# ZJU-FAST-Lab/Dftpav

Hardware: AMD Instinct MI355X
Metric: trajectory solves/sec (batched), 16-piece MINCO (higher is better)
Workload: dtype f64

## Files before the change

### dftpav_amd/csrc/quad_common.h

```cpp
#pragma once
#include "ref_order_common.h"

namespace dftpav {
namespace reford {

__device__ __forceinline__ double row_chain16(double acc, double v) {
  const double one = 1.0;
  asm volatile("s_nop 1\n\t" DFTPAV_FMAC_BCAST16 : "+v"(acc) : "v"(v), "v"(one));
  return acc;
}
__device__ __forceinline__ double row_add_lane0(double acc, double v) {
  const double one = 1.0;
  asm volatile("s_nop 1\n\t" DFTPAV_FMAC_BCAST(0) : "+v"(acc) : "v"(v), "v"(one));
  return acc;
}
__device__ __forceinline__ double row_max16(double v) {
  v = fmax(v, mov_dpp<0xB1>(v));
  v = fmax(v, mov_dpp<0x4E>(v));
  v = fmax(v, mov_dpp<0x141>(v));
  v = fmax(v, mov_dpp<0x140>(v));
  return v;
}
template <int CTRL> __device__ __forceinline__ double nb_dpp(double v) {
  int lo = __double2loint(v), hi = __double2hiint(v);
  lo = __builtin_amdgcn_update_dpp(0, lo, CTRL, 0xf, 0xf, true);
  hi = __builtin_amdgcn_update_dpp(0, hi, CTRL, 0xf, 0xf, true);
  return __hiloint2double(hi, lo);
}


constexpr int kDense = 24;
static_assert(kDense <= 32, "a lane's slots of the list are the bits of a 32-bit mask (solver_ref4.hip: mine |= 1u << e)");
struct DenseLds {
  ldsi_t id;
  ldsd_t s1;
  ldsd_t pl;
  ldsd_t out;
};
__host__ __device__ inline size_t q4_dense_bytes() { return ((size_t)kDense * (4 + 8 + 32 + 120) + 15) & ~(size_t)15; }
__device__ inline void q4_carve_dense(DenseLds &d, char *base) {
  ldsd_t p = (ldsd_t)reinterpret_cast<double *>(base);
  d.s1 = p; p += kDense;
  d.pl = p; p += 4 * kDense;
  d.out = p; p += 15 * kDense;
  d.id = (ldsi_t)p;
}

}
}
```

### dftpav_amd/csrc/solver_ref4.hip

```cpp
#include <hip/hip_runtime.h>
#include <cstdio>
#include <cstdlib>
#include <algorithm>

#include "ref_order_common.h"
#include "quad_common.h"

namespace dftpav {
namespace reford {

constexpr int kQPool = 64;
static_assert(kQPool <= 64 && kQPool % 8 == 0, "a lane's pool slots are the bits of a 64-bit mask; the chain pass reads the permutation eight bytes at a time");
typedef unsigned char __attribute__((address_space(3))) *ldsb_t;
typedef const unsigned long long __attribute__((address_space(3))) *ldscu64_t;
#ifndef DFTPAV_Q4_WAVES_PER_EU
#define DFTPAV_Q4_WAVES_PER_EU 1
#endif
constexpr int kQ4WavesPerCU = 4 * DFTPAV_Q4_WAVES_PER_EU;

struct Q4 {
  ldsd_t xs, gs;
  ldsd_t bnd;
  ldsd_t tw;
  ldsd_t st;
  ldsd_t alpha;
  ldsd_t pool;
  ldsb_t perm;
  ldsi_t ist;
};
__host__ __device__ inline size_t q4_team_doubles(int mem) { return 32 + 32 + 12 + 6 + sNUM + (size_t)mem + kQPool * 3 + kQPool / 8; }
__host__ __device__ inline size_t q4_team_bytes(int mem) { return (q4_team_doubles(mem) * sizeof(double) + iNUM * sizeof(int) + 15) & ~(size_t)15; }
__host__ __device__ inline size_t q4_shared_bytes(int N) { return ((size_t)pk_segment_doubles(N) * sizeof(double) + 15) & ~(size_t)15; }
__device__ inline void q4_carve(Q4 &q, char *team, int mem) {
  ldsd_t p = (ldsd_t)reinterpret_cast<double *>(team);
  q.xs = p; p += 32;
  q.gs = p; p += 32;
  q.bnd = p; p += 12;
  q.tw = p; p += 6;
  q.st = p; p += sNUM;
  q.alpha = p; p += mem;
  q.pool = p; p += kQPool * 3;
  q.perm = (ldsb_t)p; p += kQPool / 8;
  q.ist = (ldsi_t)p;
}

__device__ __forceinline__ double row_sum32(double p0, double p1, int n, int l) {
  double acc = row_chain16(0.0, l < n ? p0 : -0.0);
  if (n > 16) acc = row_chain16(acc, 16 + l < n ? p1 : -0.0);
  return acc;
}
template <int Q>
__device__ __forceinline__ void sweep4(ldscd_t tab, double (&bq)[12], int N, int l) {
  constexpr bool DESC = Q == 1 || Q == 3, DIV = Q == 1 || Q == 2;
  ldscd_t ip = tab + 48;
  v2d_t c[pk_size(Q) / 2];
  {
    const int sl = DESC ? N - 1 - l : l;
    const int bi = sl >= 1 && sl <= N - 2 ? sl - 1 : 0;
    const ldscv2_t a = (ldscv2_t)(ip + bi * pk_size(Q));
    if (N > 2) {
#pragma unroll
      for (int u = 0; u < pk_size(Q) / 2; u++) c[u] = a[u];
    } else {
#pragma unroll
      for (int u = 0; u < pk_size(Q) / 2; u++) c[u] = v2d_t{0.0, 0.0};
    }
  }
#pragma unroll 1
  for (int s = 0; s < N; s++) {
    const int p = DESC ? N - 1 - s : s;
    double w[6][2];
#pragma unroll
    for (int r = 0; r < 6; r++)
#pragma unroll
      for (int d = 0; d < 2; d++) {
        w[r][d] = DESC ? nb_dpp<0x101>(bq[2 * (5 - r) + d]) : nb_dpp<0x111>(bq[2 * r + d]);
      }
    if (s == 0 || s == N - 1) {
      const ldscv2_t a = (ldscv2_t)(s == 0 ? tab : ip + (N - 2) * pk_size(Q));
      if (s == 0) {
#pragma unroll
        for (int r = 0; r < 6; r++) w[r][0] = w[r][1] = 0.0;
      }
      if (l == p) {
#pragma unroll
        for (int r = 0; r < 6; r++) {
          v2d_t ce[4];
#pragma unroll
          for (int u = 0; u < 4; u++) ce[u] = a[4 * r + u];
          const int rr = DESC ? 5 - r : r;
#pragma unroll
          for (int d = 0; d < 2; d++) {
            double acc = bq[2 * rr + d];
#pragma unroll
            for (int k = 0; k < 6; k++) {
              const double ck = (k & 1) ? ce[k >> 1].y : ce[k >> 1].x;
              const double t = ck * w[(r + k) % 6][d];
              acc = ck != 0.0 ? acc - t : acc;
            }
            if (DIV) acc = div_by_rcp(acc, ce[3].x, ce[3].y);
            w[r][d] = acc;
            bq[2 * rr + d] = acc;
          }
        }
      }
    } else {
      if (l == p) {
        auto at = [&](int o) { return (o & 1) ? c[o >> 1].y : c[o >> 1].x; };
#pragma unroll
        for (int r = 0; r < 6; r++) {
          const int rr = DESC ? 5 - r : r;
#pragma unroll
          for (int d = 0; d < 2; d++) {
            double acc = bq[2 * rr + d];
#pragma unroll
            for (int k = 0; k < 6; k++)
              if (pk_mask(Q, r) & (1 << k)) acc = acc - at(pk_off(Q, r, k)) * w[(r + k) % 6][d];
            if (DIV) acc = div_by_rcp(acc, at(pk_diag0(Q) + 2 * r), at(pk_diag0(Q) + 2 * r + 1));
            w[r][d] = acc;
            bq[2 * rr + d] = acc;
          }
        }
      }
    }
  }
}

__device__ __forceinline__ void q4_split(const double (&bq)[12], double (&X)[6], double (&Y)[6], int l) {
  const bool lo = (l & 8) == 0;
#pragma unroll
  for (int r = 0; r < 6; r++) {
    const double own = bq[2 * r], far = nb_dpp<0x128>(bq[2 * r + 1]);
    X[r] = lo ? own : far;
    Y[r] = lo ? far : own;
  }
}
__device__ __forceinline__ void q4_unsplit(const double (&X)[6], const double (&Y)[6], double (&bq)[12], int l) {
  const bool lo = (l & 8) == 0;
#pragma unroll
  for (int r = 0; r < 6; r++) {
    bq[2 * r] = lo ? X[r] : Y[r];
    bq[2 * r + 1] = nb_dpp<0x128>(lo ? Y[r] : X[r]);
  }
}
template <int Q>
__device__ __forceinline__ void sweep4_split(ldscd_t tab, double (&X)[6], double (&Y)[6], int l) {
  constexpr bool DESC = Q == 1 || Q == 3, DIV = Q == 1 || Q == 2;
  constexpr int N = 16;
  ldscd_t ip = tab + 48;
  const int l8 = l & 7;
  auto fetch = [&](const double (&R)[6], double (&w)[6]) {
#pragma unroll
    for (int r = 0; r < 6; r++) w[r] = DESC ? nb_dpp<0x101>(R[5 - r]) : nb_dpp<0x111>(R[r]);
  };
  auto end_step = [&](double (&R)[6], double (&w)[6], ldscv2_t a) {
    v2d_t cb[6][4];
#pragma unroll
    for (int r = 0; r < 6; r++)
#pragma unroll
      for (int u = 0; u < (DIV ? 4 : 3); u++) cb[r][u] = a[4 * r + u];
    asm volatile("" ::: "memory");
#pragma unroll
    for (int r = 0; r < 6; r++) {
      const v2d_t(&ce)[4] = cb[r];
      const int rr = DESC ? 5 - r : r;
      double acc = R[rr];
#pragma unroll
      for (int k = 0; k < 6; k++) {
        const double ck = (k & 1) ? ce[k >> 1].y : ce[k >> 1].x;
        const double t = ck * w[(r + k) % 6];
        acc = ck != 0.0 ? acc - t : acc;
      }
      if (DIV) acc = div_by_rcp(acc, ce[3].x, ce[3].y);
      w[r] = acc;
      R[rr] = acc;
    }
  };
  auto interior = [&](double (&R)[6], int s1, double (&w)[6]) {
    v2d_t c[pk_size(Q) / 2];
    {
      const int sl = (s1 & 8) + (DESC ? 7 - l8 : l8);
      const int bi = sl >= 1 && sl <= N - 2 ? sl - 1 : 0;
      const ldscv2_t a = (ldscv2_t)(ip + bi * pk_size(Q));
#pragma unroll
      for (int u = 0; u < pk_size(Q) / 2; u++) c[u] = a[u];
    }
    auto at = [&](int o) { return (o & 1) ? c[o >> 1].y : c[o >> 1].x; };
#pragma unroll 1
    for (int s = s1; s < s1 + 7; s++) {
      const bool own = l8 == ((DESC ? N - 1 - s : s) & 7);
      if (own) {
#pragma unroll
        for (int r = 0; r < 6; r++) {
          const int rr = DESC ? 5 - r : r;
          double acc = R[rr];
#pragma unroll
// ... 480 lines not shown
    if (l == 0) q.ist[iRET] = -1005;
    return false;
  }
  if (l == 0) {
    q.st[sFINIT] = q.st[sFX];
    q.st[sDGINIT] = dginit;
    q.st[sDGTEST] = P.f_dec_coeff * dginit;
    q.st[sDSTEST] = P.s_curv_coeff * dginit;
    q.st[sMU] = 0.0;
    q.st[sNU] = P.max_step;
    q.st[sSTP] = step;
    q.ist[iCOUNT] = 0;
    q.ist[iBRACKT] = 0;
    q.ist[iTOUCHED] = 0;
  }
  if (e0) q.xs[l] = v.xp0 + step * v.d0;
  if (e1) q.xs[16 + l] = v.xp1 + step * v.d1;
  return true;
}

constexpr int kQB = 8;
constexpr int kQNpad = 64;
static_assert(kQuadMirrorRows == 2 * kQB, "DevBatch::histM holds kQB rows of either end of a ring");
template <bool Y3> struct QBlk {
  d2_t a[kQB], b[kQB];
  d2_t yr[Y3 ? kQB : 1];
};
typedef double __attribute__((ext_vector_type(2))) qd2_t;

#define DFTPAV_FMAC_BCAST15 \
  DFTPAV_FMAC_BCAST(0) DFTPAV_FMAC_BCAST(1) DFTPAV_FMAC_BCAST(2) DFTPAV_FMAC_BCAST(3) DFTPAV_FMAC_BCAST(4) DFTPAV_FMAC_BCAST(5) DFTPAV_FMAC_BCAST(6) \
  DFTPAV_FMAC_BCAST(7) DFTPAV_FMAC_BCAST(8) DFTPAV_FMAC_BCAST(9) DFTPAV_FMAC_BCAST(10) DFTPAV_FMAC_BCAST(11) DFTPAV_FMAC_BCAST(12) \
  DFTPAV_FMAC_BCAST(13) DFTPAV_FMAC_BCAST(14)
__device__ __forceinline__ double row_chain15(double acc, double v) {
  const double one = 1.0;
  asm volatile("s_nop 1\n\t" DFTPAV_FMAC_BCAST15 : "+v"(acc) : "v"(v), "v"(one));
  return acc;
}
template <bool Y3> __device__ __forceinline__ double q4_rec_sum(double p0, double p1, int n) {
  double acc = row_chain16(0.0, p0);
  if (n > 16) acc = Y3 ? row_chain16(acc, p1) : row_chain15(acc, p1);
  return acc;
}

template <int DIR, bool Y3>
__device__ __forceinline__ void q4_load_blk(QBlk<Y3> &R, gcd2_t hS, gcd2_t hM, gcd2_t hR, int m, int l, int &jl) {
  const bool wrap = DIR < 0 ? jl < kQB - 1 : jl > m - kQB;
  const int mr = DIR < 0 ? kQB + jl : jl - (m - kQB);
  const gcd2_t row = (wrap ? hM + mr * kQNpad : hS + jl * kQNpad) + l;
#pragma unroll
  for (int u = 0; u < kQB; u++) {
    R.a[u] = row[DIR * u * kQNpad];
    R.b[u] = row[DIR * u * kQNpad + 16];
  }
  if (Y3) {
    int jr = jl;
#pragma unroll
    for (int u = 0; u < kQB; u++) {
      R.yr[Y3 ? u : 0] = hR[jr];
      if (DIR < 0) jr = jr == 0 ? m - 1 : jr - 1;
      else jr = jr == m - 1 ? 0 : jr + 1;
    }
  }
  if (DIR < 0) {
    jl -= kQB;
    jl = jl < 0 ? jl + m : jl;
  } else {
    jl += kQB;
    jl = jl >= m ? jl - m : jl;
  }
}
template <bool Y3> __device__ __forceinline__ void q4_pin_blk(QBlk<Y3> &R) {
#pragma unroll
  for (int u = 0; u < kQB; u++) {
    asm volatile("" : "+v"(R.a[u].x), "+v"(R.a[u].y), "+v"(R.b[u].x), "+v"(R.b[u].y));
    if (Y3) asm volatile("" : "+v"(R.yr[Y3 ? u : 0].x), "+v"(R.yr[Y3 ? u : 0].y));
  }
}
template <bool Y3> __device__ __forceinline__ d2_t q4_blk_yr(const QBlk<Y3> &R, int u) {
  if (Y3) return R.yr[Y3 ? u : 0];
  d2_t yr;
  yr.x = mov_dpp<0x15F>(R.b[u].x);
  yr.y = mov_dpp<0x15F>(R.b[u].y);
  return yr;
}
template <bool EXACT, bool Y3>
__device__ __forceinline__ void q4_first_steps(const QBlk<Y3> &R, ldsd_t al, int i0, int bound, int n, int l, bool exact, double &d0, double &d1) {
#pragma unroll
  for (int u = 0; u < kQB; u++) {
    if (i0 + u < bound) {
      const d2_t yr = q4_blk_yr<Y3>(R, u);
      const double dot = q4_rec_sum<Y3>(R.a[u].x * d0, R.b[u].x * d1, n);
      const double a = EXACT && exact ? dot / yr.x : div_by_rcp<false>(dot, yr.x, yr.y);
      if (l == 0) al[u] = a;
      const double na = -a;
      d0 = d0 + na * R.a[u].y;
      d1 = d1 + na * R.b[u].y;
    }
  }
}
template <bool EXACT, bool Y3>
__device__ __forceinline__ void q4_second_steps(const QBlk<Y3> &R, ldscd_t al, int i0, int bound, int n, int l, bool exact, double &d0, double &d1) {
#pragma unroll
  for (int u = 0; u < kQB; u++) {
    if (i0 + u < bound) {
      const double av = al[kQB - 1 - u];
      const d2_t yr = q4_blk_yr<Y3>(R, u);
      const double dot = q4_rec_sum<Y3>(R.a[u].y * d0, R.b[u].y * d1, n);
      const double beta = EXACT && exact ? dot / yr.x : div_by_rcp<false>(dot, yr.x, yr.y);
      const double cf = av - beta;
      d0 = d0 + cf * R.a[u].x;
      d1 = d1 + cf * R.b[u].x;
    }
  }
}
template <bool EXACT, bool Y3>
__device__ __forceinline__ void q4_two_loop(const Q4 &q, gcd2_t hS, gcd2_t hM, gcd2_t hR, int m, int n, int l, int bound, int ne, bool exact, double sc0, double &d0,
                                            double &d1) {
  QBlk<Y3> A, B;
  int jl = ne == 0 ? m - 1 : ne - 1;
  q4_load_blk<-1>(A, hS, hM, hR, m, l, jl);
#pragma unroll 1
  for (int i0 = 0; i0 < bound; i0 += 2 * kQB) {
    q4_pin_blk(A);
    q4_load_blk<-1>(B, hS, hM, hR, m, l, jl);
    q4_first_steps<EXACT>(A, q.alpha + i0, i0, bound, n, l, exact, d0, d1);
    q4_pin_blk(B);
    q4_load_blk<-1>(A, hS, hM, hR, m, l, jl);
    q4_first_steps<EXACT>(B, q.alpha + (i0 + kQB), i0 + kQB, bound, n, l, exact, d0, d1);
  }
  d0 = d0 * sc0;
  d1 = d1 * sc0;
  __builtin_amdgcn_fence(__ATOMIC_SEQ_CST, "wavefront");
  jl = ne - bound;
  jl = jl < 0 ? jl + m : jl;
  q4_load_blk<+1>(A, hS, hM, hR, m, l, jl);
#pragma unroll 1
  for (int i0 = 0; i0 < bound; i0 += 2 * kQB) {
    const ldscd_t al = (ldscd_t)(q.alpha + (bound - kQB - i0));
    q4_pin_blk(A);
    q4_load_blk<+1>(B, hS, hM, hR, m, l, jl);
    q4_second_steps<EXACT>(A, al, i0, bound, n, l, exact, d0, d1);
    q4_pin_blk(B);
    q4_load_blk<+1>(A, hS, hM, hR, m, l, jl);
    q4_second_steps<EXACT>(B, al - kQB, i0 + kQB, bound, n, l, exact, d0, d1);
  }
}
__device__ __forceinline__ void q4_store_pair(gd_t hS, gd_t hM, int m, int end, int e, d2_t v) {
  ((gd2_t)hS)[(size_t)end * kQNpad + e] = v;
  if (end < kQB) ((gd2_t)hM)[(kQB + end) * kQNpad + e] = v;
  if (end >= m - kQB) ((gd2_t)hM)[(end - (m - kQB)) * kQNpad + e] = v;
}

__device__ __forceinline__ void q4_advance(const DevBatch &D, const Q4 &q, QVec &v, double f, gd_t hS, gd_t hM, gd_t hR, int l, Prof &pr) {
  const DevParams &P = D.P;
  const int n = D.L.n, m = P.mem_size;
  const bool e0 = l < n, e1 = 16 + l < n;
  int action = kActEval;
  if (q.ist[iPHASE] == 0) {
    const double g0 = e0 ? q.gs[l] : 0.0, g1 = e1 ? q.gs[16 + l] : 0.0;
    const double x0 = e0 ? q.xs[l] : 0.0, x1 = e1 ? q.xs[16 + l] : 0.0;
    v.d0 = e0 ? -g0 : 0.0;
    v.d1 = e1 ? -g1 : 0.0;
    const double gmax = row_max16(fmax(fabs(g0), fabs(g1))), xmax = row_max16(fmax(fabs(x0), fabs(x1)));
    const double dd = row_sum32((-g0) * (-g0), (-g1) * (-g1), n, l);
    __builtin_amdgcn_fence(__ATOMIC_SEQ_CST, "wavefront");
    if (l == 0) {
      q.st[sFX] = f;
      q.st[sPF0] = f;
      q.ist[iEVALS] = 1;
      q.ist[iEND] = 0;
      q.ist[iBOUND] = 0;
      q.ist[iHISTLO] = 0;
      q.ist[iHISTHI] = 0;
      q.ist[iPHASE] = 1;
    }
    if (gmax / fmax(1.0, xmax) < P.g_epsilon) {
      if (l == 0) {
        q.ist[iRET] = 0;
        q.ist[iK] = 0;
      }
      action = kActDone;
    } else {
      if (l == 0) {
        q.st[sSTEP] = 1.0 / sqrt(dd);
        q.ist[iK] = 1;
      }
      __threadfence_block();
      if (!q4_begin_iteration(P, q, v, n, l)) action = kActDone;
    }
    if (l == 0) q.ist[iACTION] = action;
    return;
  }

  const double fx = f;
  const double finit = q.st[sFINIT];
  double stp = q.st[sSTP];
  const int count = q.ist[iCOUNT] + 1;
  int ls = 0;
  bool decided = false;
  const int evals_before = q.ist[iEVALS];
  __threadfence_block();
  if (l == 0) {
    q.st[sFX] = fx;
    q.ist[iEVALS] = evals_before + 1;
    q.ist[iCOUNT] = count;
  }
  if (isinf(fx) || isnan(fx)) {
    ls = -1012;
    decided = true;
  } else if (P.past > 0 && fabs(finit - fx) / (fabs(finit) + 1.0) < P.delta / P.past) {
    ls = count;
    decided = true;
  } else {
    double mu = q.st[sMU], nu = q.st[sNU];
    bool brackt = q.ist[iBRACKT] != 0;
    const int touched = q.ist[iTOUCHED];
    if (fx > finit + stp * q.st[sDGTEST]) {
      nu = stp;
      brackt = true;
    } else {
      const double g0 = e0 ? q.gs[l] : 0.0, g1 = e1 ? q.gs[16 + l] : 0.0;
      const double gs = row_sum32(g0 * v.d0, g1 * v.d1, n, l);
      if (gs < q.st[sDSTEST]) {
        mu = stp;
      } else {
        ls = count;
        decided = true;
      }
    }
    bool touch_now = false;
    if (!decided) {
      if (P.max_linesearch <= count) {
        ls = -1009;
        decided = true;
      } else if (brackt && (nu - mu) < P.machine_prec * nu) {
        ls = -1007;
        decided = true;
      } else {
        if (brackt) stp = 0.5 * (mu + nu);
        else stp *= 2.0;
        if (stp < P.min_step) {
          ls = -1011;
          decided = true;
        } else if (stp > P.max_step) {
          if (touched) {
            ls = -1010;
            decided = true;
          } else {
            touch_now = true;
            stp = P.max_step;
          }
        }
      }
    }
    __threadfence_block();
    if (l == 0) {
      q.st[sMU] = mu;
      q.st[sNU] = nu;
      q.ist[iBRACKT] = brackt ? 1 : 0;
      q.st[sSTP] = stp;
      if (touch_now) q.ist[iTOUCHED] = 1;
    }
    if (!decided) {
      if (e0) q.xs[l] = v.xp0 + stp * v.d0;
      if (e1) q.xs[16 + l] = v.xp1 + stp * v.d1;
      if (l == 0) q.ist[iACTION] = kActEval;
      pr.tick(6);
      return;
    }
  }
  if (l == 0) q.st[sSTEP] = stp;
  if (ls < 0) {
    if (e0) {
      q.xs[l] = v.xp0;
      q.gs[l] = v.gp0;
    }
    if (e1) {
      q.xs[16 + l] = v.xp1;
      q.gs[16 + l] = v.gp1;
    }
    if (l == 0) {
      q.ist[iRET] = ls;
      q.ist[iACTION] = kActDone;
    }
    return;
  }

  const double x0 = e0 ? q.xs[l] : 0.0, x1 = e1 ? q.xs[16 + l] : 0.0;
  const double g0 = e0 ? q.gs[l] : 0.0, g1 = e1 ? q.gs[16 + l] : 0.0;
  int k = q.ist[iK];
  {
    const double gmax = row_max16(fmax(fabs(g0), fabs(g1))), xmax = row_max16(fmax(fabs(x0), fabs(x1)));
    const int kGoOn = 12345;
    int ret = kGoOn;
    if (gmax / fmax(1.0, xmax) < P.g_epsilon) {
      ret = 0;
    } else {
      if (0 < P.past) {
        const int slot = k % P.past;
        const double pf = q.st[sPF0 + slot];
        __threadfence_block();
        if (P.past <= k) {
          const double rate = fabs(pf - fx) / fmax(1.0, fabs(fx));
          if (rate < P.delta) ret = 1;
        }
        if (ret == kGoOn && l == 0) q.st[sPF0 + slot] = fx;
      }
      if (ret == kGoOn && P.max_iterations != 0 && P.max_iterations <= k) ret = -1008;
    }
    if (ret != kGoOn) {
      if (l == 0) {
        q.ist[iRET] = ret;
        q.ist[iACTION] = kActDone;
      }
      return;
    }
  }
  ++k;
  pr.tick(6);
  const int end = q.ist[iEND];
  int bound = q.ist[iBOUND];
  __threadfence_block();
  if (l == 0) q.ist[iK] = k;

  const double sv0 = e0 ? x0 - v.xp0 : 0.0, sv1 = e1 ? x1 - v.xp1 : 0.0;
  const double yv0 = e0 ? g0 - v.gp0 : 0.0, yv1 = e1 ? g1 - v.gp1 : 0.0;
  if (e0) {
    d2_t sy;
    sy.x = sv0;
    sy.y = yv0;
    q4_store_pair(hS, hM, m, end, l, sy);
  }
  if (e1) {
    d2_t sy;
    sy.x = sv1;
    sy.y = yv1;
    q4_store_pair(hS, hM, m, end, 16 + l, sy);
  }
  v.d0 = e0 ? -g0 : 0.0;
  v.d1 = e1 ? -g1 : 0.0;
  const double ys = row_sum32(yv0 * sv0, yv1 * sv1, n, l);
  const double yy = row_sum32(yv0 * yv0, yv1 * yv1, n, l);
  const double ss = row_sum32(sv0 * sv0, sv1 * sv1, n, l);
  const double gpgp = row_sum32(v.gp0 * v.gp0, v.gp1 * v.gp1, n, l);
  if (l == 0) {
    d2_t yr;
    yr.x = ys;
    yr.y = 1.0 / ys;
    ((gd2_t)hR)[end] = yr;
    if (!rcp_route_ok(ys)) q.ist[iSLOWDIV] = 1;
  }
  const bool y3 = n > 31;
  if (l == 15 && !y3) {
    d2_t yr;
    yr.x = ys;
    yr.y = 1.0 / ys;
    q4_store_pair(hS, hM, m, end, 31, yr);
  }
  const double cau = ss * sqrt(gpgp) * P.cautious_factor;
  pr.tick(7);
  if (ys > cau) {
    ++bound;
    bound = m < bound ? m : bound;
    const int ne = end + 1 == m ? 0 : end + 1;
    __threadfence_block();
    const bool exact = q.ist[iSLOWDIV] != 0;
    double d0 = v.d0, d1 = v.d1;
    const gcd2_t cS = (gcd2_t)hS, cM = (gcd2_t)hM, cR = (gcd2_t)hR;
    if (__builtin_amdgcn_ballot_w64(exact) != 0ull) {
      if (y3) q4_two_loop<true, true>(q, cS, cM, cR, m, n, l, bound, ne, exact, ys / yy, d0, d1);
      else q4_two_loop<true, false>(q, cS, cM, cR, m, n, l, bound, ne, exact, ys / yy, d0, d1);
    } else {
      if (y3) q4_two_loop<false, true>(q, cS, cM, cR, m, n, l, bound, ne, exact, ys / yy, d0, d1);
      else q4_two_loop<false, false>(q, cS, cM, cR, m, n, l, bound, ne, exact, ys / yy, d0, d1);
    }
    v.d0 = e0 ? d0 : 0.0;
    v.d1 = e1 ? d1 : 0.0;
    if (l == 0) {
      q.ist[iEND] = ne;
      q.ist[iBOUND] = bound;
      long long hs = ((long long)q.ist[iHISTHI] << 32) | (unsigned int)q.ist[iHISTLO];
      hs += bound;
      q.ist[iHISTLO] = (int)(hs & 0xffffffffLL);
      q.ist[iHISTHI] = (int)(hs >> 32);
    }
  }
  if (l == 0) q.st[sSTEP] = 1.0;
  pr.tick(8);
  __threadfence_block();
  const bool ok = q4_begin_iteration(P, q, v, n, l);
  if (l == 0) q.ist[iACTION] = ok ? kActEval : kActDone;
  pr.tick(6);
}

__device__ inline void q4_state_io(const DevBatch &D, const Q4 &q, QVec &v, int b, int l, bool save) {
  const int n = D.L.n, npad = D.L.npad;
  double *rec = D.state + (size_t)b * D.state_stride;
  for (int h = 0; h < 2; h++) {
    const int e = 16 * h + l;
    if (e >= n) {
      if (!save) {
        q.xs[e] = 0.0;
        q.gs[e] = 0.0;
        if (h == 0) { v.xp0 = 0.0; v.gp0 = 0.0; v.d0 = 0.0; } else { v.xp1 = 0.0; v.gp1 = 0.0; v.d1 = 0.0; }
      }
      continue;
    }
    if (save) {
      rec[0 * npad + e] = q.xs[e];
      rec[1 * npad + e] = h == 0 ? v.xp0 : v.xp1;
      rec[2 * npad + e] = q.gs[e];
      rec[3 * npad + e] = h == 0 ? v.gp0 : v.gp1;
      rec[4 * npad + e] = h == 0 ? v.d0 : v.d1;
    } else {
      q.xs[e] = rec[0 * npad + e];
      q.gs[e] = rec[2 * npad + e];
      if (h == 0) {
        v.xp0 = rec[1 * npad + e];
        v.gp0 = rec[3 * npad + e];
        v.d0 = rec[4 * npad + e];
      } else {
        v.xp1 = rec[1 * npad + e];
        v.gp1 = rec[3 * npad + e];
        v.d1 = rec[4 * npad + e];
      }
    }
  }
  double *r2 = rec + 5 * npad;
  for (int w = l; w < sNUM; w += 16) {
    if (save) r2[w] = q.st[w];
    else q.st[w] = r2[w];
  }
  int *ri = reinterpret_cast<int *>(r2 + 24);
  for (int w = l; w < iNUM; w += 16) {
    if (save) ri[w] = q.ist[w];
    else q.ist[w] = ri[w];
  }
}

template <bool FAST, bool RECT>
__global__ void __launch_bounds__(256, DFTPAV_Q4_WAVES_PER_EU)
    ref4_kernel(const DevBatch *__restrict__ Dp, int mode, const double *__restrict__ tabs, const double *__restrict__ cor_t, double *__restrict__ scratch, int source,
                int slice, int hand) {
  extern __shared__ double lds_raw[];
  const DevBatch &D = *Dp;
  const DevLayout &L = D.L;
  const int tidb = threadIdx.x, Tb = blockDim.x, lane = tidb & 63, wv = tidb >> 6, W = Tb >> 6, row = lane >> 4, l = lane & 15;
  const int n = L.n, N = L.Ntot, H = L.H, mem = D.P.mem_size;
  Q4 q;
  q4_carve(q, reinterpret_cast<char *>(lds_raw) + q4_shared_bytes(N) + (size_t)(wv * 4 + row) * q4_team_bytes(mem), mem);
  DenseLds dl;
  q4_carve_dense(dl, reinterpret_cast<char *>(lds_raw) + q4_shared_bytes(N) + (size_t)W * 4 * q4_team_bytes(mem) + (size_t)wv * q4_dense_bytes());
  const ldscd_t tab = (ldscd_t)lds_raw;
  for (int i = tidb; i < pk_segment_doubles(N); i += Tb) ((ldsd_t)lds_raw)[i] = tabs[i];
  __syncthreads();
  const bool ring = mode == kModeSolve && (source & 1) != 0;
  const bool force_exact_div = (source & 2) != 0;
  const int nterm = 5 * H + 4, JP = L.Kmax + 1;
  const size_t cpitch = (size_t)JP * 16;
  const size_t scratch_per_traj = (size_t)L.Npts * nterm * kRec + (size_t)L.Npts * nterm;
  Prof pr;
  pr.on = false;
  pr.acc = nullptr;
  pr.last = 0;
  QVec v{0.0, 0.0, 0.0, 0.0, 0.0, 0.0};
  int b = -1;
  bool act = false, resumed = false;
  long long tick0 = 0;
  int steps = 0;

  for (int pass = 0;; pass++) {
    if (!act) {
      int id = -1;
      if (ring) {
        for (int r = 0; r < 4; r++)
          if (row == r && l == 0) id = ring_pop(D.qctl, D.queue, D.qcap);
        id = __shfl(id, lane & 48);
      } else if (pass == 0) {
        id = ((int)blockIdx.x * W + wv) * 4 + row;
        if (id >= D.B) id = -1;
      }
      if (id >= 0) {
        b = id;
        act = true;
        resumed = ring && D.sflag[b] == 1;
        if (resumed) {
          q4_state_io(D, q, v, b, l, false);
        } else {
          const double *xsrc = (mode == kModeSolve) ? D.x0 : D.x_in;
          for (int h = 0; h < 2; h++) {
            const int e = 16 * h + l;
            q.xs[e] = e < n ? xsrc[(size_t)b * n + e] : 0.0;
            q.gs[e] = 0.0;
          }
          v = QVec{0.0, 0.0, 0.0, 0.0, 0.0, 0.0};
          q.ist[l] = (l == iSLOWDIV && force_exact_div) ? 1 : 0;
        }
        if (l < 12) q.bnd[l] = l < 6 ? D.iniS[(size_t)b * 6 + l] : D.finS[(size_t)b * 6 + (l - 6)];
        tick0 = wall_clock64();
        pr.start(D.prof != nullptr && mode == kModeSolve && l == 0, D.prof + (size_t)b * 12, resumed);
        __builtin_amdgcn_fence(__ATOMIC_SEQ_CST, "wavefront");
      }
    }
    if (__builtin_amdgcn_ballot_w64(act) == 0ull) break;
    if (act) {
      const gcd_t cor = RECT ? (gcd_t)(cor_t + ((size_t)b * JP * 80 + l) * 2) : (gcd_t)(cor_t + (size_t)b * L.H * 4 * cpitch + l);
      const gd_t ovf = (gd_t)(scratch + (size_t)b * scratch_per_traj);
      const double f = q4_eval<FAST, RECT>(D, q, dl, tab, cor, cpitch, ovf, l, pr);
      if (mode == kModeEval) {
        for (int h = 0; h < 2; h++) {
          const int e = 16 * h + l;
          if (e < n) D.g_out[(size_t)b * n + e] = q.gs[e];
        }
        if (l == 0) D.f_eval[b] = f;
        act = false;
      } else {
        const gd_t hS = (gd_t)(D.histS + (size_t)b * mem * kQNpad * 2);
        const gd_t hM = (gd_t)(D.histM + (size_t)b * kQuadMirrorRows * kQNpad * 2);
        const gd_t hR = (gd_t)(D.histR + (size_t)b * mem * 2);
        q4_advance(D, q, v, f, hS, hM, hR, l, pr);
        __builtin_amdgcn_fence(__ATOMIC_SEQ_CST, "wavefront");
        if (q.ist[iACTION] == kActDone) {
          for (int h = 0; h < 2; h++) {
            const int e = 16 * h + l;
            if (e < n) D.x_out[(size_t)b * n + e] = q.xs[e];
          }
          if (l == 0) {
            const double fx = q.st[sFX];
            const int ret = q.ist[iRET];
            D.f_out[b] = fx;
            D.status[b] = ret;
            D.iters[b] = q.ist[iK];
            D.evals[b] = q.ist[iEVALS];
            D.hist_sum[b] = ((long long)q.ist[iHISTHI] << 32) | (unsigned int)q.ist[iHISTLO];
            {
              double *rec = reinterpret_cast<double *>(D.records + (size_t)16 * b);
              rec[0] = fx;
              int *ri = reinterpret_cast<int *>(rec + 1);
              ri[0] = ret;
              ri[1] = q.ist[iK];
            }
            if (D.records_host != nullptr) {
              double *rh = reinterpret_cast<double *>(D.records_host + (size_t)16 * b);
              rh[0] = fx;
              int *rj = reinterpret_cast<int *>(rh + 1);
              rj[0] = ret;
              rj[1] = q.ist[iK];
            }
            D.ticks[b] = (resumed ? D.ticks[b] : 0) + (wall_clock64() - tick0);
            int ok = (ret == 0 || ret == 1 || ret == 2 || ret == -1008 || ret == -1009) ? 1 : 0;
            if (fx >= D.P.fail_cost) ok = 0;
            D.success[b] = ok;
            if (ring) {
              D.sflag[b] = 2;
              atomicSub(&D.qctl[3], 1u);
            }
          }
          act = false;
        }
      }
    }
    if (!ring) {
      if (mode == kModeEval) break;
      continue;
    }
    steps++;
    if (slice > 0 && steps >= slice) {
      steps = 0;
      const bool leave = hand > 0 && __hip_atomic_load(&D.qctl[3], __ATOMIC_RELAXED, __HIP_MEMORY_SCOPE_AGENT) <= (unsigned)hand;
      if (act) {
        q4_state_io(D, q, v, b, l, true);
        __threadfence();
        if (l == 0) {
          D.ticks[b] = (resumed ? D.ticks[b] : 0) + (wall_clock64() - tick0);
          D.sflag[b] = 1;
        }
      }
      for (int r = 0; r < 4; r++)
        if (act && row == r && l == 0) ring_push(D.qctl, D.queue, D.qcap, b);
      act = false;
      if (leave) break;
    }
  }
}

__global__ void q4_corridor_kernel(const double *__restrict__ cor, double *__restrict__ out, int B, int H4, int NptsPad, int N, int K, int Kd, int JP) {
  const size_t total = (size_t)B * H4 * JP * 16;
  for (size_t i = (size_t)blockIdx.x * blockDim.x + threadIdx.x; i < total; i += (size_t)gridDim.x * blockDim.x) {
    const int p = (int)(i & 15);
    const size_t r = i >> 4;
    const int j = (int)(r % JP);
    const size_t bc = r / JP;
    double v = 0.0;
    if (p < N) {
      const int Kp = (p == 0 || p == N - 1) ? Kd : K;
      const int pt0 = p == 0 ? 0 : (Kd + 1) + (p - 1) * (K + 1);
      if (j <= Kp) v = cor[bc * NptsPad + pt0 + j];
    }
    out[i] = v;
  }
}

__global__ void q4_rect_check_kernel(const double *__restrict__ cor, int B, int Npts, int NptsPad, int *__restrict__ flag) {
  const size_t total = (size_t)B * Npts;
  const unsigned long long sign = 0x8000000000000000ull;
  for (size_t i = (size_t)blockIdx.x * blockDim.x + threadIdx.x; i < total; i += (size_t)gridDim.x * blockDim.x) {
    const size_t b = i / Npts;
    const int pt = (int)(i % Npts);
    const double *c = cor + b * 16 * NptsPad + pt;
    unsigned long long n[4][2];
    for (int k = 0; k < 4; k++)
      for (int q = 0; q < 2; q++) n[k][q] = (unsigned long long)__double_as_longlong(c[(size_t)(4 * k + q) * NptsPad]);
    const unsigned long long C = n[1][0], S = n[1][1];
    const bool nan = (C & ~sign) > 0x7ff0000000000000ull || (S & ~sign) > 0x7ff0000000000000ull;
    const bool ok = !nan && n[0][0] == (S ^ sign) && n[0][1] == C && n[2][0] == S && n[2][1] == (C ^ sign) && n[3][0] == (C ^ sign) && n[3][1] == (S ^ sign);
    if (!ok) *flag = 1;
  }
}

__global__ void q4_corridor_rect_kernel(const double *__restrict__ cor, d2_t *__restrict__ out, int B, int NptsPad, int N, int K, int Kd, int JP) {
  const size_t total = (size_t)B * JP * 80;
  for (size_t i = (size_t)blockIdx.x * blockDim.x + threadIdx.x; i < total; i += (size_t)gridDim.x * blockDim.x) {
    const int p = (int)(i & 15);
    const int u = (int)((i >> 4) % 5);
    const size_t r = i / 80;
    const int j = (int)(r % JP);
    const size_t b = r / JP;
    d2_t v = {0.0, 0.0};
    if (p < N) {
      const int Kp = (p == 0 || p == N - 1) ? Kd : K;
      const int pt0 = p == 0 ? 0 : (Kd + 1) + (p - 1) * (K + 1);
      if (j <= Kp) {
        const int c0 = u == 0 ? 4 : 4 * (u - 1) + 2;
        const double *src = cor + (b * 16 + c0) * NptsPad + pt0 + j;
        v.x = src[0];
        v.y = src[NptsPad];
      }
    }
    out[i] = v;
  }
}

}

bool reference_order_quad_supported(const DevLayout &L, const DevParams &P, int S) {
  if (L.M != 1 || S != 0 || L.n > 32 || L.Ntot > 16 || L.Ntot < 2 || L.H < 1 || L.H > 5) return false;
  if (L.npad != reford::kQNpad || P.mem_size < reford::kQB) return false;
  return reford::q4_shared_bytes(L.Ntot) + 4 * reford::q4_team_bytes(P.mem_size) + reford::q4_dense_bytes() <= 160 * 1024;
}
size_t reference_order_quad_corridor_doubles(const DevLayout &L, int B) { return (size_t)B * L.H * 4 * (L.Kmax + 1) * 16; }
QuadSizes reference_order_quad_sizes(const DevLayout &L, const DevParams &P) {
  return {reford::q4_shared_bytes(L.Ntot), reford::q4_team_bytes(P.mem_size) + (reford::q4_dense_bytes() + 3) / 4, reford::kQ4WavesPerCU, 768};
}
hipError_t launch_quad_corridor(const DevBatch &D, double *cor_t, bool rect, hipStream_t stream) {
  const DevLayout &L = D.L;
  const size_t total = rect ? (size_t)D.B * (L.Kmax + 1) * 80 : reference_order_quad_corridor_doubles(L, D.B);
  const int grid = (int)std::min<size_t>((total + 255) / 256, 65536);
  if (rect)
    hipLaunchKernelGGL(reford::q4_corridor_rect_kernel, dim3(grid), dim3(256), 0, stream, D.corridor, reinterpret_cast<reford::d2_t *>(cor_t), D.B, D.NptsPad, L.Ntot, L.K,
                       L.Kd, L.Kmax + 1);
  else
    hipLaunchKernelGGL(reford::q4_corridor_kernel, dim3(grid), dim3(256), 0, stream, D.corridor, cor_t, D.B, L.H * 4, D.NptsPad, L.Ntot, L.K, L.Kd, L.Kmax + 1);
  return hipGetLastError();
}
hipError_t launch_quad_rect_check(const double *corridor, int B, int Npts, int NptsPad, int *d_flag, hipStream_t stream) {
  hipError_t e = hipMemsetAsync(d_flag, 0, sizeof(int), stream);
  if (e != hipSuccess) return e;
  const size_t total = (size_t)B * Npts;
  const int grid = (int)std::min<size_t>((total + 255) / 256, 65536);
  hipLaunchKernelGGL(reford::q4_rect_check_kernel, dim3(grid), dim3(256), 0, stream, corridor, B, Npts, NptsPad, d_flag);
  return hipGetLastError();
}
QuadKernel ref4_kernel_for(bool fast, bool rect) {
  if (fast && rect) return &reford::ref4_kernel<true, true>;
  return fast ? &reford::ref4_kernel<true, false> : &reford::ref4_kernel<false, false>;
}

}
```

Baseline: 45250.

## Decouple wave rows from trajectories via per-wave context pool and phase-split L-BFGS step

Each wave now holds kQCtx trajectory contexts in LDS, and its four 16-lane rows are scheduled each pass onto contexts needing either an objective evaluation or the two-loop recursion. This lets rows stay busy when trajectories sit in different phases. q4_advance is split into an eval-side part and a recursion part so the two can be batched separately. The per-row scratch (alpha, pool, dense buffers) is shared across contexts as a union, which keeps LDS within budget. In exchange it adds scheduling ballots, context save/restore through LDS, and more complicated ring draining.

```diff
diff --git a/dftpav_amd/csrc/quad_common.h b/dftpav_amd/csrc/quad_common.h
--- a/dftpav_amd/csrc/quad_common.h
+++ b/dftpav_amd/csrc/quad_common.h
@@ -37,7 +37,7 @@
   ldsd_t pl;
   ldsd_t out;
 };
-__host__ __device__ inline size_t q4_dense_bytes() { return ((size_t)kDense * (4 + 8 + 32 + 120) + 15) & ~(size_t)15; }
+__host__ __device__ constexpr size_t q4_dense_bytes() { return ((size_t)kDense * (4 + 8 + 32 + 120) + 15) & ~(size_t)15; }
 __device__ inline void q4_carve_dense(DenseLds &d, char *base) {
   ldsd_t p = (ldsd_t)reinterpret_cast<double *>(base);
   d.s1 = p; p += kDense;
diff --git a/dftpav_amd/csrc/solver_ref4.hip b/dftpav_amd/csrc/solver_ref4.hip
--- a/dftpav_amd/csrc/solver_ref4.hip
+++ b/dftpav_amd/csrc/solver_ref4.hip
@@ -18,30 +18,57 @@
 #endif
 constexpr int kQ4WavesPerCU = 4 * DFTPAV_Q4_WAVES_PER_EU;
 
+#ifndef DFTPAV_Q4_CTX
+#define DFTPAV_Q4_CTX 4
+#endif
+constexpr int kQCtx = DFTPAV_Q4_CTX;
+static_assert(kQCtx >= 4 && kQCtx <= 16, "the rows of a wave take four contexts at a time; a context's state is read by the lane of its number");
+enum { kCtxFree = 0, kCtxEval = 1, kCtxRecur = 2 };
+enum { mB = 0, mRESUMED, mNEED, mSINCE, mNUM = 4 };
+enum { sSC0 = sENERGY + 1 };
+static_assert(sSC0 < sNUM, "a free slot of the scalar state");
+typedef long long __attribute__((address_space(3))) *ldsll_t;
+
 struct Q4 {
   ldsd_t xs, gs;
   ldsd_t bnd;
+  ldsd_t st;
+  ldsd_t vec;
+  ldsi_t ist;
+  ldsi_t meta;
+  ldsll_t clk;
   ldsd_t tw;
-  ldsd_t st;
-  ldsd_t alpha;
   ldsd_t pool;
   ldsb_t perm;
-  ldsi_t ist;
+  ldsd_t alpha;
 };
-__host__ __device__ inline size_t q4_team_doubles(int mem) { return 32 + 32 + 12 + 6 + sNUM + (size_t)mem + kQPool * 3 + kQPool / 8; }
-__host__ __device__ inline size_t q4_team_bytes(int mem) { return (q4_team_doubles(mem) * sizeof(double) + iNUM * sizeof(int) + 15) & ~(size_t)15; }
-__host__ __device__ inline size_t q4_shared_bytes(int N) { return ((size_t)pk_segment_doubles(N) * sizeof(double) + 15) & ~(size_t)15; }
-__device__ inline void q4_carve(Q4 &q, char *team, int mem) {
-  ldsd_t p = (ldsd_t)reinterpret_cast<double *>(team);
+__host__ __device__ constexpr size_t q4_ctx_bytes() { return (size_t)(32 + 32 + 12 + sNUM + 6 * 16) * sizeof(double) + (iNUM + mNUM) * sizeof(int) + 2 * sizeof(long long); }
+__host__ __device__ constexpr size_t q4_row_bytes() { return (size_t)(6 + kQPool * 3 + kQPool / 8) * sizeof(double); }
+static_assert(q4_ctx_bytes() % 16 == 0 && q4_row_bytes() % 16 == 0, "16-byte units");
+__host__ __device__ constexpr size_t q4_work_bytes(int mem) {
+  const size_t ev = 4 * q4_row_bytes() + q4_dense_bytes(), rc = (size_t)4 * mem * sizeof(double);
+  return ((ev > rc ? ev : rc) + 15) & ~(size_t)15;
+}
+__host__ __device__ constexpr size_t q4_wave_bytes(int mem) { return kQCtx * q4_ctx_bytes() + q4_work_bytes(mem); }
+__host__ __device__ constexpr size_t q4_shared_bytes(int N) { return ((size_t)pk_segment_doubles(N) * sizeof(double) + 15) & ~(size_t)15; }
+static_assert(q4_shared_bytes(16) + q4_wave_bytes(256) <= 160 * 1024 / kQ4WavesPerCU, "kQCtx contexts per wave keep four workgroups on a CU at mem = 256, N = 16");
+__device__ inline void q4_carve_ctx(Q4 &q, char *ctx) {
+  ldsd_t p = (ldsd_t)reinterpret_cast<double *>(ctx);
   q.xs = p; p += 32;
   q.gs = p; p += 32;
   q.bnd = p; p += 12;
+  q.st = p; p += sNUM;
+  q.vec = p; p += 6 * 16;
+  q.clk = (ldsll_t)p; p += 2;
+  q.ist = (ldsi_t)p;
+  q.meta = q.ist + iNUM;
+}
+__device__ inline void q4_carve_row(Q4 &q, char *work, int row, int mem) {
+  ldsd_t p = (ldsd_t)reinterpret_cast<double *>(work + (size_t)row * q4_row_bytes());
   q.tw = p; p += 6;
-  q.st = p; p += sNUM;
-  q.alpha = p; p += mem;
   q.pool = p; p += kQPool * 3;
-  q.perm = (ldsb_t)p; p += kQPool / 8;
-  q.ist = (ldsi_t)p;
+  q.perm = (ldsb_t)p;
+  q.alpha = (ldsd_t)reinterpret_cast<double *>(work) + (size_t)row * mem;
 }
 
 __device__ __forceinline__ double row_sum32(double p0, double p1, int n, int l) {
@@ -828,7 +855,7 @@
   if (end >= m - kQB) ((gd2_t)hM)[(end - (m - kQB)) * kQNpad + e] = v;
 }
 
-__device__ __forceinline__ void q4_advance(const DevBatch &D, const Q4 &q, QVec &v, double f, gd_t hS, gd_t hM, gd_t hR, int l, Prof &pr) {
+__device__ __forceinline__ int q4_advance_a(const DevBatch &D, const Q4 &q, QVec &v, double f, gd_t hS, gd_t hM, gd_t hR, int l, Prof &pr) {
   const DevParams &P = D.P;
   const int n = D.L.n, m = P.mem_size;
   const bool e0 = l < n, e1 = 16 + l < n;
@@ -866,7 +893,7 @@
       if (!q4_begin_iteration(P, q, v, n, l)) action = kActDone;
     }
     if (l == 0) q.ist[iACTION] = action;
-    return;
+    return action == kActDone ? kCtxFree : kCtxEval;
   }
 
   const double fx = f;
@@ -943,7 +970,7 @@
       if (e1) q.xs[16 + l] = v.xp1 + stp * v.d1;
       if (l == 0) q.ist[iACTION] = kActEval;
       pr.tick(6);
-      return;
+      return kCtxEval;
     }
   }
   if (l == 0) q.st[sSTEP] = stp;
@@ -960,7 +987,7 @@
       q.ist[iRET] = ls;
       q.ist[iACTION] = kActDone;
     }
-    return;
+    return kCtxFree;
   }
 
   const double x0 = e0 ? q.xs[l] : 0.0, x1 = e1 ? q.xs[16 + l] : 0.0;
@@ -990,13 +1017,12 @@
         q.ist[iRET] = ret;
         q.ist[iACTION] = kActDone;
       }
-      return;
+      return kCtxFree;
     }
   }
   ++k;
   pr.tick(6);
   const int end = q.ist[iEND];
-  int bound = q.ist[iBOUND];
   __threadfence_block();
   if (l == 0) q.ist[iK] = k;
 
@@ -1037,6 +1063,27 @@
   const double cau = ss * sqrt(gpgp) * P.cautious_factor;
   pr.tick(7);
   if (ys > cau) {
+    if (l == 0) q.st[sSC0] = ys / yy;
+    return kCtxRecur;
+  }
+  if (l == 0) q.st[sSTEP] = 1.0;
+  pr.tick(8);
+  __threadfence_block();
+  const bool ok = q4_begin_iteration(P, q, v, n, l);
+  if (l == 0) q.ist[iACTION] = ok ? kActEval : kActDone;
+  pr.tick(6);
+  return ok ? kCtxEval : kCtxFree;
+}
+__device__ __forceinline__ int q4_advance_b(const DevBatch &D, const Q4 &q, QVec &v, gd_t hS, gd_t hM, gd_t hR, int l, Prof &pr) {
+  const DevParams &P = D.P;
+  const int n = D.L.n, m = P.mem_size;
+  const bool e0 = l < n, e1 = 16 + l < n;
+  pr.tick(10);
+  const int end = q.ist[iEND];
+  int bound = q.ist[iBOUND];
+  const double sc0 = q.st[sSC0];
+  const bool y3 = n > 31;
+  {
     ++bound;
     bound = m < bound ? m : bound;
     const int ne = end + 1 == m ? 0 : end + 1;
@@ -1045,11 +1092,11 @@
     double d0 = v.d0, d1 = v.d1;
     const gcd2_t cS = (gcd2_t)hS, cM = (gcd2_t)hM, cR = (gcd2_t)hR;
     if (__builtin_amdgcn_ballot_w64(exact) != 0ull) {
-      if (y3) q4_two_loop<true, true>(q, cS, cM, cR, m, n, l, bound, ne, exact, ys / yy, d0, d1);
-      else q4_two_loop<true, false>(q, cS, cM, cR, m, n, l, bound, ne, exact, ys / yy, d0, d1);
+      if (y3) q4_two_loop<true, true>(q, cS, cM, cR, m, n, l, bound, ne, exact, sc0, d0, d1);
+      else q4_two_loop<true, false>(q, cS, cM, cR, m, n, l, bound, ne, exact, sc0, d0, d1);
     } else {
-      if (y3) q4_two_loop<false, true>(q, cS, cM, cR, m, n, l, bound, ne, exact, ys / yy, d0, d1);
-      else q4_two_loop<false, false>(q, cS, cM, cR, m, n, l, bound, ne, exact, ys / yy, d0, d1);
+      if (y3) q4_two_loop<false, true>(q, cS, cM, cR, m, n, l, bound, ne, exact, sc0, d0, d1);
+      else q4_two_loop<false, false>(q, cS, cM, cR, m, n, l, bound, ne, exact, sc0, d0, d1);
     }
     v.d0 = e0 ? d0 : 0.0;
     v.d1 = e1 ? d1 : 0.0;
@@ -1068,6 +1115,18 @@
   const bool ok = q4_begin_iteration(P, q, v, n, l);
   if (l == 0) q.ist[iACTION] = ok ? kActEval : kActDone;
   pr.tick(6);
+  return ok ? kCtxEval : kCtxFree;
+}
+
+__device__ __forceinline__ void q4_vec_load(const Q4 &q, QVec &v, int l) {
+  v.xp0 = q.vec[0 * 16 + l]; v.xp1 = q.vec[1 * 16 + l];
+  v.gp0 = q.vec[2 * 16 + l]; v.gp1 = q.vec[3 * 16 + l];
+  v.d0 = q.vec[4 * 16 + l]; v.d1 = q.vec[5 * 16 + l];
+}
+__device__ __forceinline__ void q4_vec_store(const Q4 &q, const QVec &v, int l) {
+  q.vec[0 * 16 + l] = v.xp0; q.vec[1 * 16 + l] = v.xp1;
+  q.vec[2 * 16 + l] = v.gp0; q.vec[3 * 16 + l] = v.gp1;
+  q.vec[4 * 16 + l] = v.d0; q.vec[5 * 16 + l] = v.d1;
 }
 
 __device__ inline void q4_state_io(const DevBatch &D, const Q4 &q, QVec &v, int b, int l, bool save) {
@@ -1124,140 +1183,245 @@
   const DevLayout &L = D.L;
   const int tidb = threadIdx.x, Tb = blockDim.x, lane = tidb & 63, wv = tidb >> 6, W = Tb >> 6, row = lane >> 4, l = lane & 15;
   const int n = L.n, N = L.Ntot, H = L.H, mem = D.P.mem_size;
+  char *const ctx0 = reinterpret_cast<char *>(lds_raw) + q4_shared_bytes(N) + (size_t)wv * q4_wave_bytes(mem);
+  char *const work = ctx0 + kQCtx * q4_ctx_bytes();
   Q4 q;
-  q4_carve(q, reinterpret_cast<char *>(lds_raw) + q4_shared_bytes(N) + (size_t)(wv * 4 + row) * q4_team_bytes(mem), mem);
+  q4_carve_ctx(q, ctx0);
+  q4_carve_row(q, work, row, mem);
   DenseLds dl;
-  q4_carve_dense(dl, reinterpret_cast<char *>(lds_raw) + q4_shared_bytes(N) + (size_t)W * 4 * q4_team_bytes(mem) + (size_t)wv * q4_dense_bytes());
+  q4_carve_dense(dl, work + 4 * q4_row_bytes());
   const ldscd_t tab = (ldscd_t)lds_raw;
   for (int i = tidb; i < pk_segment_doubles(N); i += Tb) ((ldsd_t)lds_raw)[i] = tabs[i];
+  if (lane < kQCtx) {
+    Q4 c;
+    q4_carve_ctx(c, ctx0 + (size_t)lane * q4_ctx_bytes());
+    c.meta[mNEED] = kCtxFree;
+    c.meta[mSINCE] = 0;
+  }
   __syncthreads();
   const bool ring = mode == kModeSolve && (source & 1) != 0;
   const bool force_exact_div = (source & 2) != 0;
   const int nterm = 5 * H + 4, JP = L.Kmax + 1;
   const size_t cpitch = (size_t)JP * 16;
   const size_t scratch_per_traj = (size_t)L.Npts * nterm * kRec + (size_t)L.Npts * nterm;
-  Prof pr;
-  pr.on = false;
-  pr.acc = nullptr;
-  pr.last = 0;
-  QVec v{0.0, 0.0, 0.0, 0.0, 0.0, 0.0};
-  int b = -1;
-  bool act = false, resumed = false;
-  long long tick0 = 0;
+  const bool prof_on = D.prof != nullptr && mode == kModeSolve && l == 0;
   int steps = 0;
+  bool drain = false;
+
+  auto take_trajectory = [&](int b) {
+    const bool resumed = ring && D.sflag[b] == 1;
+    if (resumed) {
+      QVec v;
+      q4_state_io(D, q, v, b, l, false);
+      q4_vec_store(q, v, l);
+    } else {
+      const double *xsrc = (mode == kModeSolve) ? D.x0 : D.x_in;
+      for (int h = 0; h < 2; h++) {
+        const int e = 16 * h + l;
+        q.xs[e] = e < n ? xsrc[(size_t)b * n + e] : 0.0;
+        q.gs[e] = 0.0;
+      }
+      q4_vec_store(q, QVec{0.0, 0.0, 0.0, 0.0, 0.0, 0.0}, l);
+      q.ist[l] = (l == iSLOWDIV && force_exact_div) ? 1 : 0;
+    }
+    if (l < 12) q.bnd[l] = l < 6 ? D.iniS[(size_t)b * 6 + l] : D.finS[(size_t)b * 6 + (l - 6)];
+    Prof pr;
+    pr.start(prof_on, D.prof + (size_t)b * 12, resumed);
+    if (l == 0) {
+      q.meta[mB] = b;
+      q.meta[mRESUMED] = resumed ? 1 : 0;
+      q.clk[0] = wall_clock64();
+      q.clk[1] = pr.last;
+    }
+  };
+  auto deal = [&](unsigned &t) {
+    int mine = -1;
+#pragma unroll
+    for (int r = 0; r < 4; r++) {
+      const int c = t != 0u ? __builtin_ctz(t) : -1;
+      t &= t - 1u;
+      mine = row == r ? c : mine;
+    }
+    return mine;
+  };
 
   for (int pass = 0;; pass++) {
-    if (!act) {
-      int id = -1;
-      if (ring) {
+    int need = kCtxFree, since = 0;
+    auto look = [&]() {
+      __builtin_amdgcn_fence(__ATOMIC_SEQ_CST, "wavefront");
+      if (lane < kQCtx) {
+        Q4 c;
+        q4_carve_ctx(c, ctx0 + (size_t)lane * q4_ctx_bytes());
+        need = c.meta[mNEED];
+        since = c.meta[mSINCE];
+      }
+    };
+    look();
+    if (ring ? !drain : pass == 0) {
+      unsigned fr = (unsigned)__builtin_amdgcn_ballot_w64(lane < (ring ? kQCtx : 4) && need == kCtxFree);
+      bool dry = false;
+      while (fr != 0u && !dry) {
+        const int c = deal(fr);
+        int id = -1;
+        if (ring) {
+          for (int r = 0; r < 4; r++)
+            if (row == r && l == 0 && c >= 0) id = ring_pop(D.qctl, D.queue, D.qcap);
+          id = __shfl(id, lane & 48);
+        } else if (c >= 0) {
+          id = ((int)blockIdx.x * W + wv) * 4 + row;
+          if (id >= D.B) id = -1;
+        }
+        if (c >= 0 && id >= 0) {
+          q4_carve_ctx(q, ctx0 + (size_t)c * q4_ctx_bytes());
+          take_trajectory(id);
+          if (l == 0) {
+            q.meta[mNEED] = kCtxEval;
+            q.meta[mSINCE] = pass;
+          }
+        }
+        dry = __builtin_amdgcn_ballot_w64(c >= 0 && id < 0) != 0ull;
+      }
+      look();
+    }
+    unsigned mE = (unsigned)__builtin_amdgcn_ballot_w64(need == kCtxEval), mR = (unsigned)__builtin_amdgcn_ballot_w64(need == kCtxRecur);
+    const int nE = __builtin_popcount(mE), nR = __builtin_popcount(mR);
+    if (!drain && nE + nR == 0) break;
+
+    if (drain && nR == 0) {
+      drain = false;
+      steps = 0;
+      const bool leave = hand > 0 && __hip_atomic_load(&D.qctl[3], __ATOMIC_RELAXED, __HIP_MEMORY_SCOPE_AGENT) <= (unsigned)hand;
+      while (mE != 0u) {
+        const int c = deal(mE);
+        int b = -1;
+        if (c >= 0) {
+          q4_carve_ctx(q, ctx0 + (size_t)c * q4_ctx_bytes());
+          b = q.meta[mB];
+          QVec v;
+          q4_vec_load(q, v, l);
+          q4_state_io(D, q, v, b, l, true);
+          __threadfence();
+          if (l == 0) {
+            D.ticks[b] = (q.meta[mRESUMED] != 0 ? D.ticks[b] : 0) + (wall_clock64() - q.clk[0]);
+            D.sflag[b] = 1;
+            q.meta[mNEED] = kCtxFree;
+          }
+        }
         for (int r = 0; r < 4; r++)
-          if (row == r && l == 0) id = ring_pop(D.qctl, D.queue, D.qcap);
-        id = __shfl(id, lane & 48);
-      } else if (pass == 0) {
-        id = ((int)blockIdx.x * W + wv) * 4 + row;
-        if (id >= D.B) id = -1;
-      }
-      if (id >= 0) {
-        b = id;
-        act = true;
-        resumed = ring && D.sflag[b] == 1;
-        if (resumed) {
-          q4_state_io(D, q, v, b, l, false);
-        } else {
-          const double *xsrc = (mode == kModeSolve) ? D.x0 : D.x_in;
+          if (c >= 0 && row == r && l == 0) ring_push(D.qctl, D.queue, D.qcap, b);
+      }
+      if (leave) break;
+      continue;
+    }
+
+    const bool recur = nR > 0 && (drain || nE == 0 || (nE < 4 && nR >= nE));
+    int mc = -1;
+    {
+      unsigned cand = recur ? mR : mE;
+#pragma unroll 1
+      for (int r = 0; r < 4 && cand != 0u; r++) {
+        int best = -1, bs = 0;
+        for (unsigned t = cand; t != 0u; t &= t - 1u) {
+          const int c = __builtin_ctz(t);
+          const int sc = __builtin_amdgcn_readlane(since, c);
+          if (best < 0 || sc < bs) {
+            best = c;
+            bs = sc;
+          }
+        }
+        cand &= ~(1u << best);
+        mc = row == r ? best : mc;
+      }
+    }
+    if (!recur) steps++;
+
+    if (mc >= 0) {
+      q4_carve_ctx(q, ctx0 + (size_t)mc * q4_ctx_bytes());
+      const int b = q.meta[mB];
+      Prof pr;
+      pr.on = prof_on;
+      pr.acc = D.prof + (size_t)b * 12;
+      pr.last = q.clk[1];
+      const gd_t hS = (gd_t)(D.histS + (size_t)b * mem * kQNpad * 2);
+      const gd_t hM = (gd_t)(D.histM + (size_t)b * kQuadMirrorRows * kQNpad * 2);
+      const gd_t hR = (gd_t)(D.histR + (size_t)b * mem * 2);
+      int nxt = recur ? kCtxRecur : kCtxEval;
+      if (!recur) {
+        const gcd_t cor = RECT ? (gcd_t)(cor_t + ((size_t)b * JP * 80 + l) * 2) : (gcd_t)(cor_t + (size_t)b * L.H * 4 * cpitch + l);
+        const gd_t ovf = (gd_t)(scratch + (size_t)b * scratch_per_traj);
+        const double f = q4_eval<FAST, RECT>(D, q, dl, tab, cor, cpitch, ovf, l, pr);
+        if (mode == kModeEval) {
           for (int h = 0; h < 2; h++) {
             const int e = 16 * h + l;
-            q.xs[e] = e < n ? xsrc[(size_t)b * n + e] : 0.0;
-            q.gs[e] = 0.0;
+            if (e < n) D.g_out[(size_t)b * n + e] = q.gs[e];
           }
-          v = QVec{0.0, 0.0, 0.0, 0.0, 0.0, 0.0};
-          q.ist[l] = (l == iSLOWDIV && force_exact_div) ? 1 : 0;
-        }
-        if (l < 12) q.bnd[l] = l < 6 ? D.iniS[(size_t)b * 6 + l] : D.finS[(size_t)b * 6 + (l - 6)];
-        tick0 = wall_clock64();
-        pr.start(D.prof != nullptr && mode == kModeSolve && l == 0, D.prof + (size_t)b * 12, resumed);
-        __builtin_amdgcn_fence(__ATOMIC_SEQ_CST, "wavefront");
-      }
-    }
-    if (__builtin_amdgcn_ballot_w64(act) == 0ull) break;
-    if (act) {
-      const gcd_t cor = RECT ? (gcd_t)(cor_t + ((size_t)b * JP * 80 + l) * 2) : (gcd_t)(cor_t + (size_t)b * L.H * 4 * cpitch + l);
-      const gd_t ovf = (gd_t)(scratch + (size_t)b * scratch_per_traj);
-      const double f = q4_eval<FAST, RECT>(D, q, dl, tab, cor, cpitch, ovf, l, pr);
-      if (mode == kModeEval) {
+          if (l == 0) D.f_eval[b] = f;
+          nxt = kCtxFree;
+        } else {
+          QVec v;
+          q4_vec_load(q, v, l);
+          nxt = q4_advance_a(D, q, v, f, hS, hM, hR, l, pr);
+          q4_vec_store(q, v, l);
+        }
+      }
+      if (nxt == kCtxRecur && (recur || !ring)) {
+        const unsigned long long inb = __builtin_amdgcn_ballot_w64(true);
+        if (prof_on && (lane & 48) == (__builtin_ctzll(inb) & 48))
+          pr.count(9, (1ll << 32) + (__builtin_popcountll(inb) == 64 ? 1ll << 48 : 0ll));
+        QVec v;
+        q4_vec_load(q, v, l);
+        nxt = q4_advance_b(D, q, v, hS, hM, hR, l, pr);
+        q4_vec_store(q, v, l);
+      }
+      __builtin_amdgcn_fence(__ATOMIC_SEQ_CST, "wavefront");
+      if (nxt == kCtxFree && mode != kModeEval) {
         for (int h = 0; h < 2; h++) {
           const int e = 16 * h + l;
-          if (e < n) D.g_out[(size_t)b * n + e] = q.gs[e];
-        }
-        if (l == 0) D.f_eval[b] = f;
-        act = false;
-      } else {
-        const gd_t hS = (gd_t)(D.histS + (size_t)b * mem * kQNpad * 2);
-        const gd_t hM = (gd_t)(D.histM + (size_t)b * kQuadMirrorRows * kQNpad * 2);
-        const gd_t hR = (gd_t)(D.histR + (size_t)b * mem * 2);
-        q4_advance(D, q, v, f, hS, hM, hR, l, pr);
-        __builtin_amdgcn_fence(__ATOMIC_SEQ_CST, "wavefront");
-        if (q.ist[iACTION] == kActDone) {
-          for (int h = 0; h < 2; h++) {
-            const int e = 16 * h + l;
-            if (e < n) D.x_out[(size_t)b * n + e] = q.xs[e];
+          if (e < n) D.x_out[(size_t)b * n + e] = q.xs[e];
+        }
+        if (l == 0) {
+          const double fx = q.st[sFX];
+          const int ret = q.ist[iRET];
+          D.f_out[b] = fx;
+          D.status[b] = ret;
+          D.iters[b] = q.ist[iK];
+          D.evals[b] = q.ist[iEVALS];
+          D.hist_sum[b] = ((long long)q.ist[iHISTHI] << 32) | (unsigned int)q.ist[iHISTLO];
+          {
+            double *rec = reinterpret_cast<double *>(D.records + (size_t)16 * b);
+            rec[0] = fx;
+            int *ri = reinterpret_cast<int *>(rec + 1);
+            ri[0] = ret;
+            ri[1] = q.ist[iK];
           }
-          if (l == 0) {
-            const double fx = q.st[sFX];
-            const int ret = q.ist[iRET];
-            D.f_out[b] = fx;
-            D.status[b] = ret;
-            D.iters[b] = q.ist[iK];
-            D.evals[b] = q.ist[iEVALS];
-            D.hist_sum[b] = ((long long)q.ist[iHISTHI] << 32) | (unsigned int)q.ist[iHISTLO];
-            {
-              double *rec = reinterpret_cast<double *>(D.records + (size_t)16 * b);
-              rec[0] = fx;
-              int *ri = reinterpret_cast<int *>(rec + 1);
-              ri[0] = ret;
-              ri[1] = q.ist[iK];
-            }
-            if (D.records_host != nullptr) {
-              double *rh = reinterpret_cast<double *>(D.records_host + (size_t)16 * b);
-              rh[0] = fx;
-              int *rj = reinterpret_cast<int *>(rh + 1);
-              rj[0] = ret;
-              rj[1] = q.ist[iK];
-            }
-            D.ticks[b] = (resumed ? D.ticks[b] : 0) + (wall_clock64() - tick0);
-            int ok = (ret == 0 || ret == 1 || ret == 2 || ret == -1008 || ret == -1009) ? 1 : 0;
-            if (fx >= D.P.fail_cost) ok = 0;
-            D.success[b] = ok;
-            if (ring) {
-              D.sflag[b] = 2;
-              atomicSub(&D.qctl[3], 1u);
-            }
+          if (D.records_host != nullptr) {
+            double *rh = reinterpret_cast<double *>(D.records_host + (size_t)16 * b);
+            rh[0] = fx;
+            int *rj = reinterpret_cast<int *>(rh + 1);
+            rj[0] = ret;
+            rj[1] = q.ist[iK];
           }
-          act = false;
-        }
+          D.ticks[b] = (q.meta[mRESUMED] != 0 ? D.ticks[b] : 0) + (wall_clock64() - q.clk[0]);
+          int ok = (ret == 0 || ret == 1 || ret == 2 || ret == -1008 || ret == -1009) ? 1 : 0;
+          if (fx >= D.P.fail_cost) ok = 0;
+          D.success[b] = ok;
+          if (ring) {
+            D.sflag[b] = 2;
+            atomicSub(&D.qctl[3], 1u);
+          }
+        }
+      }
+      if (l == 0) {
+        q.meta[mNEED] = nxt;
+        q.meta[mSINCE] = pass;
+        q.clk[1] = pr.last;
       }
     }
     if (!ring) {
       if (mode == kModeEval) break;
       continue;
     }
-    steps++;
-    if (slice > 0 && steps >= slice) {
-      steps = 0;
-      const bool leave = hand > 0 && __hip_atomic_load(&D.qctl[3], __ATOMIC_RELAXED, __HIP_MEMORY_SCOPE_AGENT) <= (unsigned)hand;
-      if (act) {
-        q4_state_io(D, q, v, b, l, true);
-        __threadfence();
-        if (l == 0) {
-          D.ticks[b] = (resumed ? D.ticks[b] : 0) + (wall_clock64() - tick0);
-          D.sflag[b] = 1;
-        }
-      }
-      for (int r = 0; r < 4; r++)
-        if (act && row == r && l == 0) ring_push(D.qctl, D.queue, D.qcap, b);
-      act = false;
-      if (leave) break;
-    }
+    if (slice > 0 && steps >= slice) drain = true;
   }
 }
 
@@ -1323,11 +1487,11 @@
 bool reference_order_quad_supported(const DevLayout &L, const DevParams &P, int S) {
   if (L.M != 1 || S != 0 || L.n > 32 || L.Ntot > 16 || L.Ntot < 2 || L.H < 1 || L.H > 5) return false;
   if (L.npad != reford::kQNpad || P.mem_size < reford::kQB) return false;
-  return reford::q4_shared_bytes(L.Ntot) + 4 * reford::q4_team_bytes(P.mem_size) + reford::q4_dense_bytes() <= 160 * 1024;
+  return reford::q4_shared_bytes(L.Ntot) + reford::q4_wave_bytes(P.mem_size) <= 160 * 1024;
 }
 size_t reference_order_quad_corridor_doubles(const DevLayout &L, int B) { return (size_t)B * L.H * 4 * (L.Kmax + 1) * 16; }
 QuadSizes reference_order_quad_sizes(const DevLayout &L, const DevParams &P) {
-  return {reford::q4_shared_bytes(L.Ntot), reford::q4_team_bytes(P.mem_size) + (reford::q4_dense_bytes() + 3) / 4, reford::kQ4WavesPerCU, 768};
+  return {reford::q4_shared_bytes(L.Ntot), reford::q4_wave_bytes(P.mem_size) / 4, reford::kQ4WavesPerCU, 768};
 }
 hipError_t launch_quad_corridor(const DevBatch &D, double *cor_t, bool rect, hipStream_t stream) {
   const DevLayout &L = D.L;
```

New measurement: 45100. Within noise of the previous version (-0.3%).
